# SeanNaren/deepspeech.pytorch

Measured on NVIDIA H100. Metric: utterances/sec (train step, 161x1000 spectrogram), higher is better.
Workload: dtype fp16-operands(rnn)+tf32(conv/fc)

## Files before the change

deepspeech.pytorch_b200/csrc/common.cuh:

```cuda
#pragma once
#include <cuda_runtime.h>
#include <stdint.h>
#include <stdio.h>
#include <string.h>
#include <atomic>

#include "../../include/ds2_b200.h"

namespace ds2 {

void set_error(const char* fmt, ...);
extern std::atomic<long long> g_launches;
int precision();
inline bool tensor_core_mode() { return precision() != DS2_PREC_FP32; }
inline bool f16_gemm_mode() { return precision() == DS2_PREC_F16; }

inline cudaStream_t as_stream(void* s) { return reinterpret_cast<cudaStream_t>(s); }

inline int current_device() {
  int d = 0;
  (void)cudaGetDevice(&d);
  return d & 63;
}
struct DeviceOnce {
  std::atomic<unsigned long long> mask{0};
  bool first() const { return !((mask.load(std::memory_order_acquire) >> current_device()) & 1ull); }
  void done() { mask.fetch_or(1ull << current_device(), std::memory_order_release); }
};
int device_sm_count();

void note_fallback(const char* what, int rnn, int T, int B, int H, int D);

extern std::atomic<void*> g_side_stream;
int side_wait_for_workspace(const void* ws, cudaStream_t main);
int side_fork(cudaStream_t main, cudaStream_t side);
int side_mark_workspace(const void* ws, cudaStream_t side);

#define DS2_CHECK_CUDA(expr)                                                             \
  do {                                                                                   \
    cudaError_t _e = (expr);                                                             \
    if (_e != cudaSuccess) {                                                             \
      ds2::set_error("%s:%d %s -> %s", __FILE__, __LINE__, #expr, cudaGetErrorString(_e)); \
      return DS2_ERR_CUDA;                                                               \
    }                                                                                    \
  } while (0)

#define DS2_REQUIRE(cond, ...)                      \
  do {                                              \
    if (!(cond)) {                                  \
      ds2::set_error(__VA_ARGS__);                  \
      return DS2_ERR_INVALID;                       \
    }                                               \
  } while (0)

#define DS2_LAUNCH(kernel, grid, block, smem, stream, ...)                \
  do {                                                                    \
    kernel<<<(grid), (block), (smem), (stream)>>>(__VA_ARGS__);           \
    ds2::g_launches.fetch_add(1, std::memory_order_relaxed);              \
    DS2_CHECK_CUDA(cudaGetLastError());                                   \
  } while (0)

void prof_begin(const char* tag, cudaStream_t st);
void prof_end(cudaStream_t st);
struct ProfRange {
  cudaStream_t st;
  ProfRange(const char* tag, cudaStream_t s) : st(s) { prof_begin(tag, s); }
  ~ProfRange() { prof_end(st); }
};
#define DS2_PROF(tag, st) ds2::ProfRange _prof_range_##__LINE__(tag, st)

inline int cdiv(long long a, long long b) { return (int)((a + b - 1) / b); }
#ifdef __CUDACC__
__device__ __forceinline__ int cdiv_dev(int a, int b) { return (a + b - 1) / b; }
#endif
inline size_t align_up(size_t x, size_t a) { return (x + a - 1) / a * a; }

template <typename T>
inline T* carve(void* base, size_t& off, size_t bytes) {
  T* at = base ? reinterpret_cast<T*>(static_cast<char*>(base) + off) : nullptr;
  off += align_up(bytes, 256);
  return at;
}

#ifdef __CUDACC__
__device__ __forceinline__ float sigmoidf_(float x) { return 1.0f / (1.0f + expf(-x)); }

__device__ __forceinline__ float warp_sum(float v) {
#pragma unroll
  for (int o = 16; o > 0; o >>= 1) v += __shfl_xor_sync(0xffffffffu, v, o);
  return v;
}
__device__ __forceinline__ double warp_sum_d(double v) {
#pragma unroll
  for (int o = 16; o > 0; o >>= 1) v += __shfl_xor_sync(0xffffffffu, v, o);
  return v;
}
#endif

int gemm_simt(int transA, int transB, int M, int N, int K, float alpha, const float* A, int lda, const float* B,
              int ldb, float beta, float* C, int ldc, cudaStream_t st, void* ws = nullptr, size_t ws_bytes = 0);
size_t gemm_simt_workspace_bytes(int M, int N, int K);
int gemm_tc(int transA, int transB, int M, int N, int K, float alpha, const float* A, int lda, const float* B,
            int ldb, float beta, float* C, int ldc, void* ws, size_t ws_bytes, cudaStream_t st);
size_t gemm_tc_workspace_bytes(int transA, int transB, int M, int N, int K);
int gemm_tc_f16(int M, int N, int K, float alpha, const void* A16, int lda, const void* B16, int ldb, float beta,
                float* C, int ldc, const float* alpha_dev, cudaStream_t st);
int f32_to_f16_rows(int rows, int cols, const float* in, size_t ld_in, void* out, size_t ld_out, const float* scale_dev,
                    cudaStream_t st);
int f32_to_f16_transpose(int rows, int cols, const float* in, size_t ld_in, void* out, size_t ld_out, void* outT,
                         size_t ld_outT, const float* scale_dev, cudaStream_t st);
int pow2_scale_for(int rows, int cols, const float* x, size_t ld, unsigned int* absmax_ws, float* scale, int top,
                   cudaStream_t st);

int bn_rows_fwd(int rows, int F, const float* x, const float* gamma, const float* beta, float* rmean, float* rvar,
                int training, float momentum, float eps, float* y, float* xhat, float* mean_invstd ,
                double* ws_sums , cudaStream_t st);
int bn_rows_reapply(int rows, int F, const float* x, const float* gamma, const float* beta,
                    const float* mean_invstd, float* y, float* xhat, cudaStream_t st);
int transpose(int R, int C, const float* in, float* out, cudaStream_t st);
int transpose_strided(int R, int C, const float* in, size_t ldi, float* out, size_t ldo, cudaStream_t st);
int bn_rows_bwd(int rows, int F, const float* xhat, const float* gamma, const float* mean_invstd, const float* dy,
                float* dx, float* dgamma, float* dbeta, double* ws_sums , cudaStream_t st);

}
```

deepspeech.pytorch_b200/csrc/conv_frontend.cu:

```cuda
#include <stdlib.h>

#include "common.cuh"

namespace ds2 {

constexpr int CO = 32;
constexpr int TD = 4, TT = 64;

template <int KH, int KW, int SH, int SW>
struct ConvGeom {
  static constexpr int ROWS = (TD - 1) * SH + KH;
  static constexpr int XIN = (4 - 1) * SW + KW;
  static constexpr int XVEC = (XIN + 3) / 4;
  static constexpr int COLS = ((15 * 4 * SW + XVEC * 4) + 3) / 4 * 4;
  static constexpr int SLAB = ROWS * COLS;
  static constexpr int WTS = KH * KW * CO;
  static constexpr size_t SMEM = (size_t)(SLAB + WTS) * sizeof(float);
};

template <int KH, int KW, int SH, int SW>
__global__ void __launch_bounds__(256) conv_fwd_kernel(const float* __restrict__ in, int Cin, int Hin, int Win,
                                                       const float* __restrict__ wpk, const float* __restrict__ bias,
                                                       float* __restrict__ out, int Hout, int Wout, size_t ob,
                                                       size_t oc, size_t orow, int PH, int PW,
// ... 230 lines not shown
    du_dz[base + i] = v;
  }
  __shared__ float red[8];
  float s = warp_sum(v);
  if (threadIdx.x % 32 == 0) red[threadIdx.x / 32] = s;
  __syncthreads();
  if (threadIdx.x == 0) {
    float tot = 0.f;
    for (int w = 0; w < (int)blockDim.x / 32; ++w) tot += red[w];
    dbias_part[((size_t)c * B + b) * gridDim.x + blockIdx.x] = tot;
  }
}

__global__ void ordered_sum_kernel(int n, const float* __restrict__ part, float* __restrict__ out) {
  __shared__ float red[256];
  const float* p = part + (size_t)blockIdx.x * n;
  float s = 0.f;
  for (int i = threadIdx.x; i < n; i += 256) s += p[i];
  red[threadIdx.x] = s;
  __syncthreads();
  for (int w = 128; w > 0; w >>= 1) {
    if (threadIdx.x < w) red[threadIdx.x] += red[threadIdx.x + w];
    __syncthreads();
  }
  if (threadIdx.x == 0) out[blockIdx.x] = red[0];
}

__global__ void bn_bwd_params2d_kernel(const double* __restrict__ sums, float* __restrict__ dgamma,
                                       float* __restrict__ dbeta) {
  int c = threadIdx.x;
  if (c < CO) { dbeta[c] = (float)sums[c]; dgamma[c] = (float)sums[CO + c]; }
}

__global__ void __launch_bounds__(256) conv2_dw_kernel(int B, int T, const float* __restrict__ dz2,
                                                       const float* __restrict__ a1, float* __restrict__ dw2) {
  constexpr int D1 = DS2_CONV1_D, D2 = DS2_CONV2_D, TW = 64, AW = TW + 12;
  __shared__ __align__(16) float dsm[TW][36];
  __shared__ float asmx[AW][33];
  const int kh = blockIdx.x, b = blockIdx.y, tid = threadIdx.x;
  const int cog = tid / 32, ci = tid % 32;
  float acc[4][11];
#pragma unroll
  for (int c = 0; c < 4; ++c)
#pragma unroll
    for (int k = 0; k < 11; ++k) acc[c][k] = 0.f;
  for (int d = 0; d < D2; ++d) {
    const int r = 2 * d + kh - 10;
    if (r < 0 || r >= D1) continue;
    for (int t0 = 0; t0 < T; t0 += TW) {
      for (int idx = tid; idx < CO * TW; idx += 256) {
        int tt = idx % TW, co = idx / TW, t = t0 + tt;
        dsm[tt][co] = (t < T) ? dz2[(((size_t)b * CO + co) * D2 + d) * T + t] : 0.f;
      }
      for (int idx = tid; idx < CO * AW; idx += 256) {
        int tt = idx % AW, c2 = idx / AW, t = t0 + tt - 5;
        asmx[tt][c2] = (t >= 0 && t < T) ? a1[(((size_t)b * CO + c2) * D1 + r) * T + t] : 0.f;
      }
      __syncthreads();
#pragma unroll 1
      for (int tb = 0; tb < TW; tb += 4) {
        float win[14];
#pragma unroll
        for (int i = 0; i < 14; ++i) win[i] = asmx[tb + i][ci];
#pragma unroll
        for (int j = 0; j < 4; ++j) {
          float4 dv = *reinterpret_cast<const float4*>(&dsm[tb + j][cog * 4]);
#pragma unroll
          for (int k = 0; k < 11; ++k) {
            float a = win[j + k];
            acc[0][k] = fmaf(dv.x, a, acc[0][k]); acc[1][k] = fmaf(dv.y, a, acc[1][k]);
            acc[2][k] = fmaf(dv.z, a, acc[2][k]); acc[3][k] = fmaf(dv.w, a, acc[3][k]);
          }
        }
      }
      __syncthreads();
    }
  }
#pragma unroll
  for (int c = 0; c < 4; ++c)
#pragma unroll
    for (int k = 0; k < 11; ++k)
      atomicAdd(&dw2[((((size_t)(cog * 4 + c)) * CO + ci) * 21 + kh) * 11 + k], acc[c][k]);
}

constexpr int C1_KG = 14, C1_TW = 64, C1_XW = 2 * C1_TW + 12, C1_DSPLIT = 6;
__global__ void __launch_bounds__(128) conv1_dw_kernel(int B, int Tin, int T, const float* __restrict__ dz1,
                                                       const float* __restrict__ x, float* __restrict__ dw1) {
  constexpr int D1 = DS2_CONV1_D, F = DS2_NUM_FREQ, TW = C1_TW, XW = C1_XW;
  __shared__ __align__(16) float dsm[TW][CO];
  __shared__ float xsm[C1_KG][XW];
  const int kh0 = blockIdx.x * C1_KG, b = blockIdx.y, tid = threadIdx.x;
  const int dper = (D1 + C1_DSPLIT - 1) / C1_DSPLIT, d0 = blockIdx.z * dper, d1 = min(D1, d0 + dper);
  const int cog = tid % 8, khl = tid / 8, kh = kh0 + khl;
  const bool worker = khl < C1_KG && kh < 41;
  const int khr = worker ? khl : 0;
  float acc[4][11];
#pragma unroll
  for (int c = 0; c < 4; ++c)
#pragma unroll
    for (int k = 0; k < 11; ++k) acc[c][k] = 0.f;
  for (int d = d0; d < d1; ++d) {
    for (int t0 = 0; t0 < T; t0 += TW) {
      for (int idx = tid; idx < CO * TW; idx += 128) {
        const int tt = idx % TW, c2 = idx / TW, t = t0 + tt;
        dsm[tt][c2] = (t < T) ? dz1[(((size_t)b * CO + c2) * D1 + d) * T + t] : 0.f;
      }
      for (int idx = tid; idx < C1_KG * XW; idx += 128) {
        const int cc = idx % XW, kl = idx / XW, r = 2 * d + kh0 + kl - 20, c = 2 * t0 + cc - 5;
        xsm[kl][cc] = (kh0 + kl < 41 && r >= 0 && r < F && c >= 0 && c < Tin) ? x[((size_t)b * F + r) * Tin + c] : 0.f;
      }
      __syncthreads();
      if (worker) {
#pragma unroll 1
        for (int tb = 0; tb < TW; tb += 4) {
          float win[17];
#pragma unroll
          for (int i = 0; i < 17; ++i) win[i] = xsm[khr][2 * tb + i];
#pragma unroll
          for (int j = 0; j < 4; ++j) {
            const float4 dv = *reinterpret_cast<const float4*>(&dsm[tb + j][cog * 4]);
#pragma unroll
            for (int k = 0; k < 11; ++k) {
              const float a = win[2 * j + k];
              acc[0][k] = fmaf(dv.x, a, acc[0][k]); acc[1][k] = fmaf(dv.y, a, acc[1][k]);
              acc[2][k] = fmaf(dv.z, a, acc[2][k]); acc[3][k] = fmaf(dv.w, a, acc[3][k]);
            }
          }
        }
      }
      __syncthreads();
    }
  }
  if (worker) {
#pragma unroll
    for (int c = 0; c < 4; ++c)
#pragma unroll
      for (int k = 0; k < 11; ++k) atomicAdd(&dw1[((size_t)(cog * 4 + c) * 41 + kh) * 11 + k], acc[c][k]);
  }
}

template <int KH, int KW, int SH, int SW>
static int launch_conv(const float* in, int B, int Cin, int Hin, int Win, const float* wpk, const float* bias,
                       float* out, int Hout, int Wout, size_t ob, size_t oc, size_t orow, int PH, int PW,
                       const int32_t* out_len, double* sums, cudaStream_t st) {
  using Gm = ConvGeom<KH, KW, SH, SW>;
  auto kern = conv_fwd_kernel<KH, KW, SH, SW>;
  DS2_CHECK_CUDA(cudaFuncSetAttribute(kern, cudaFuncAttributeMaxDynamicSharedMemorySize, (int)Gm::SMEM));
  dim3 grid(cdiv(Wout, TT), cdiv(Hout, TD), B);
  DS2_LAUNCH(kern, grid, 256, Gm::SMEM, st, in, Cin, Hin, Win, wpk, bias, out, Hout, Wout, ob, oc, orow, PH, PW,
             out_len, sums);
  return DS2_OK;
}

int conv_tc_run(const float* in_cl, int B, int T, int R_in, int R_out, const float* taps, int n_taps, int J,
                int row_mul, int row_off, int row_step, int w_off, int w_step, float* out, size_t ob, size_t oc,
                size_t orow, int out_row_mul, int out_row_off, const float* bias, const int32_t* out_len,
                double* stat_sums, cudaStream_t st);
int nchw_to_cl(int B, int R, int T, const float* in, float* out, cudaStream_t st);
int pack_conv2_tc(const float* w2, float* wn_fwd, float* wd_bwd, cudaStream_t st);
int conv2_wgrad_tc(const float* dz2, const float* a1, float* a1_shifted, float* part, int B, int T, float* dw2,
                   cudaStream_t st);
int conv1_wgrad_tc(const float* dz1, const float* x, float* xs, float* part, int B, int T, int Tp, float* dw1,
                   cudaStream_t st);
size_t conv_wgrad_tc_partial_floats();

struct ConvWs {
  float *wpk1, *wpk2, *wTe, *wTo, *du2, *da1;
  float *taps_f, *taps_b, *cl;
  float* shifted;
  float* wg_part;
  float* db_part;
  double* sums;
};
static size_t conv_ws_carve(int B, int T, void* base, ConvWs& w) {
  const size_t Tp = (size_t)(T - 1) / 2 + 1;
  size_t off = 0;
  w.wpk1 = carve<float>(base, off, (size_t)41 * 11 * CO * 4);
  w.wpk2 = carve<float>(base, off, (size_t)CO * 21 * 11 * CO * 4);
  w.wTe = carve<float>(base, off, (size_t)CO * 11 * 11 * CO * 4);
  w.wTo = carve<float>(base, off, (size_t)CO * 10 * 11 * CO * 4);
  w.sums = carve<double>(base, off, 4 * 64 * sizeof(double));
  w.du2 = carve<float>(base, off, (size_t)B * CO * DS2_CONV2_D * Tp * 4);
  w.da1 = carve<float>(base, off, (size_t)B * CO * DS2_CONV1_D * Tp * 4);
  w.taps_f = carve<float>(base, off, (size_t)21 * 352 * 32 * 4);
  w.taps_b = carve<float>(base, off, (size_t)21 * 352 * 32 * 4);
  w.cl = carve<float>(base, off, (size_t)B * CO * DS2_CONV1_D * Tp * 4);
  w.shifted = carve<float>(base, off, (size_t)4 * B * CO * DS2_CONV1_D * (Tp + 4) * 4);
  w.wg_part = carve<float>(base, off, conv_wgrad_tc_partial_floats() * 4);
  w.db_part = carve<float>(base, off, (size_t)CO * B * cdiv((long long)DS2_CONV1_D * Tp, 256) * 4);
  return off;
}

}

extern "C" {
using namespace ds2;

size_t ds2_conv_frontend_workspace_bytes(int B, int T) {
  if (B <= 0 || T <= 0) return 0;
  ConvWs w;
  return conv_ws_carve(B, T, nullptr, w) + 256;
}

int ds2_conv_frontend_fwd(int B, int T, const float* x, const int32_t* out_len, const float* w1, const float* b1,
                          const float* g1, const float* be1, float* rm1, float* rv1, const float* w2,
                          const float* b2, const float* g2, const float* be2, float* rm2, float* rv2, int training,
                          float momentum, float eps, float* y, float* z1, float* a1, float* z2, float* stats,
                          void* ws, size_t ws_bytes, void* stream) {
  DS2_REQUIRE(B > 0 && T > 0, "conv fwd: bad shape B=%d T=%d", B, T);
  DS2_REQUIRE(ws_bytes >= ds2_conv_frontend_workspace_bytes(B, T), "conv fwd: workspace too small");
  cudaStream_t st = as_stream(stream);
  const int Tp = (T - 1) / 2 + 1, D1 = DS2_CONV1_D, D2 = DS2_CONV2_D, F = DS2_NUM_FREQ;
  ConvWs W;
  conv_ws_carve(B, T, ws, W);
  DS2_PROF("conv_fwd", st);
  DS2_CHECK_CUDA(cudaMemsetAsync(W.sums, 0, 4 * 64 * sizeof(double), st));
  DS2_LAUNCH(pack_fwd_kernel, cdiv(41 * 11 * CO, 256), 256, 0, st, 1, 41, 11, w1, W.wpk1);
  DS2_LAUNCH(pack_fwd_kernel, cdiv(CO * 21 * 11 * CO, 256), 256, 0, st, CO, 21, 11, w2, W.wpk2);
  int rc = launch_conv<41, 11, 2, 2>(x, B, 1, F, T, W.wpk1, b1, z1, D1, Tp, (size_t)CO * D1 * Tp, (size_t)D1 * Tp,
                                     (size_t)Tp, 20, 5, out_len, training ? W.sums : nullptr, st);
  if (rc) return rc;
  DS2_LAUNCH(bn2d_finalize_kernel, 1, 32, 0, st, (double)B * D1 * Tp, W.sums, g1, be1, rm1, rv1, training, momentum,
             eps, stats);
  DS2_LAUNCH(bn_act_kernel, 132 * 8, 256, 0, st, B, D1, Tp, z1, stats, g1, be1, out_len, a1);
  if (tensor_core_mode()) {
    rc = nchw_to_cl(B, D1, Tp, a1, W.cl, st);
    if (rc) return rc;
    rc = pack_conv2_tc(w2, W.taps_f, nullptr, st);
    if (rc) return rc;
    rc = conv_tc_run(W.cl, B, Tp, D1, D2, W.taps_f, 21, 21, 2, -10, 1, 0, 1, z2, (size_t)CO * D2 * Tp, (size_t)D2 * Tp,
                     (size_t)Tp, 1, 0, b2, out_len, training ? W.sums + 64 : nullptr, st);
  } else {
    rc = launch_conv<21, 11, 2, 1>(a1, B, CO, D1, Tp, W.wpk2, b2, z2, D2, Tp, (size_t)CO * D2 * Tp, (size_t)D2 * Tp,
                                   (size_t)Tp, 10, 5, out_len, training ? W.sums + 64 : nullptr, st);
  }
  if (rc) return rc;
  DS2_LAUNCH(bn2d_finalize_kernel, 1, 32, 0, st, (double)B * D2 * Tp, W.sums + 64, g2, be2, rm2, rv2, training,
             momentum, eps, stats + 64);
  DS2_LAUNCH(bn_act_transpose_kernel, dim3(cdiv(Tp, 32), cdiv(CO * D2, 32), B), dim3(32, 8), 0, st, B, D2, Tp, z2,
             stats + 64, g2, be2, out_len, y);
  return DS2_OK;
}

int ds2_conv_frontend_bwd(int B, int T, const float* x, const int32_t* out_len, const float* w1, const float* g1,
                          const float* be1, const float* w2, const float* g2, const float* be2, const float* z1,
                          const float* a1, const float* z2, const float* stats, const float* dy, float* dw1,
                          float* db1, float* dg1, float* dbe1, float* dw2, float* db2, float* dg2, float* dbe2,
                          void* ws, size_t ws_bytes, void* stream) {
  DS2_REQUIRE(B > 0 && T > 0, "conv bwd: bad shape B=%d T=%d", B, T);
  DS2_REQUIRE(ws_bytes >= ds2_conv_frontend_workspace_bytes(B, T), "conv bwd: workspace too small");
  (void)w1;
  cudaStream_t st = as_stream(stream);
  const int Tp = (T - 1) / 2 + 1, D1 = DS2_CONV1_D, D2 = DS2_CONV2_D;
  ConvWs W;
  conv_ws_carve(B, T, ws, W);
  double* s2 = W.sums + 128;
  double* s1 = W.sums + 192;
  DS2_PROF("conv_bwd", st);
  DS2_CHECK_CUDA(cudaMemsetAsync(s2, 0, 128 * sizeof(double), st));
  DS2_CHECK_CUDA(cudaMemsetAsync(db2, 0, CO * sizeof(float), st));
  DS2_CHECK_CUDA(cudaMemsetAsync(db1, 0, CO * sizeof(float), st));
  DS2_CHECK_CUDA(cudaMemsetAsync(dw2, 0, sizeof(float) * CO * CO * 21 * 11, st));
  DS2_CHECK_CUDA(cudaMemsetAsync(dw1, 0, sizeof(float) * CO * 41 * 11, st));

  DS2_LAUNCH(bn_bwd_reduce_kernel<true>, dim3(cdiv(Tp, 32), cdiv(CO * D2, 32), B), dim3(32, 8), 0, st, B, D2, Tp, z2,
             stats + 64, g2, be2, out_len, dy, W.du2, s2);
  DS2_LAUNCH(bn_bwd_params2d_kernel, 1, 32, 0, st, s2, dg2, dbe2);
  DS2_LAUNCH(bn_bwd_apply_kernel, dim3(cdiv(D2 * Tp, 256), CO, B), 256, 0, st, B, D2, Tp, 1.0 / ((double)B * D2 * Tp),
             z2, stats + 64, g2, out_len, s2, W.du2, W.db_part);
  DS2_LAUNCH(ordered_sum_kernel, CO, 256, 0, st, B * cdiv(D2 * Tp, 256), W.db_part, db2);
  cudaStream_t side = as_stream(g_side_stream.load());
  bool forked = false;
  {
    int wrc = 1;
    if (tensor_core_mode()) {
      cudaStream_t wst = st;
      if (side && Tp % 4 == 0) {
        int frc = side_fork(st, side);
        if (frc) return frc;
        wst = side;
        forked = true;
      }
      wrc = conv2_wgrad_tc(W.du2, a1, W.shifted, W.wg_part, B, Tp, dw2, wst);
      if (wrc < 0) return wrc;
      if (forked) {
        int mrc = side_mark_workspace(ws, side);
        if (mrc) return mrc;
      }
    }
    if (wrc == 1) DS2_LAUNCH(conv2_dw_kernel, dim3(21, B), 256, 0, st, B, Tp, W.du2, a1, dw2);
  }
  DS2_LAUNCH(pack_bwd_data_kernel, cdiv(CO * 11 * 11 * CO, 256), 256, 0, st, 0, w2, W.wTe);
  DS2_LAUNCH(pack_bwd_data_kernel, cdiv(CO * 10 * 11 * CO, 256), 256, 0, st, 1, w2, W.wTo);
  const size_t ob = (size_t)CO * D1 * Tp, oc = (size_t)D1 * Tp;
  int rc;
  if (tensor_core_mode()) {
    rc = nchw_to_cl(B, D2, Tp, W.du2, W.cl, st);
    if (rc) return rc;
    rc = pack_conv2_tc(w2, nullptr, W.taps_b, st);
    if (rc) return rc;
    rc = conv_tc_run(W.cl, B, Tp, D2, 41, W.taps_b, 21, 11, 1, 5, -1, 0, 2, W.da1, ob, oc, (size_t)Tp, 2, 0, nullptr,
                     nullptr, nullptr, st);
    if (rc) return rc;
    rc = conv_tc_run(W.cl, B, Tp, D2, 40, W.taps_b, 21, 10, 1, 5, -1, 1, 2, W.da1, ob, oc, (size_t)Tp, 2, 1, nullptr,
                     nullptr, nullptr, st);
    if (rc) return rc;
  } else {
    rc = launch_conv<11, 11, 1, 1>(W.du2, B, CO, D2, Tp, W.wTe, nullptr, W.da1, 41, Tp, ob, oc, (size_t)2 * Tp, 5, 5,
                                   nullptr, nullptr, st);
    if (rc) return rc;
    rc = launch_conv<10, 11, 1, 1>(W.du2, B, CO, D2, Tp, W.wTo, nullptr, W.da1 + Tp, 40, Tp, ob, oc, (size_t)2 * Tp, 4, 5,
                                   nullptr, nullptr, st);
    if (rc) return rc;
  }
  DS2_LAUNCH(bn_bwd_reduce_kernel<false>, dim3(cdiv(Tp, 32), cdiv(CO * D1, 32), B), dim3(32, 8), 0, st, B, D1, Tp,
             z1, stats, g1, be1, out_len, W.da1, W.da1, s1);
  DS2_LAUNCH(bn_bwd_params2d_kernel, 1, 32, 0, st, s1, dg1, dbe1);
  DS2_LAUNCH(bn_bwd_apply_kernel, dim3(cdiv(D1 * Tp, 256), CO, B), 256, 0, st, B, D1, Tp, 1.0 / ((double)B * D1 * Tp),
             z1, stats, g1, out_len, s1, W.da1, W.db_part);
  DS2_LAUNCH(ordered_sum_kernel, CO, 256, 0, st, B * cdiv(D1 * Tp, 256), W.db_part, db1);
  if (forked) {
    int jrc = side_wait_for_workspace(ws, st);
    if (jrc) return jrc;
  }
  {
    int wrc = 1;
    if (tensor_core_mode()) {
      wrc = conv1_wgrad_tc(W.da1, x, W.shifted, W.wg_part, B, T, Tp, dw1, st);
      if (wrc < 0) return wrc;
    }
    if (wrc == 1) DS2_LAUNCH(conv1_dw_kernel, dim3(3, B, C1_DSPLIT), 128, 0, st, B, T, Tp, W.da1, x, dw1);
  }
  return DS2_OK;
}

}
```

deepspeech.pytorch_b200/csrc/conv_tc.cu:

```cuda
#include "common.cuh"
#include "tc_common.cuh"

namespace ds2 {
int make_tmap_4d_f32(CUtensorMap* out, const float* base, const unsigned long long dims[4],
                     const unsigned long long strides_bytes[3], const unsigned int box[4]);
int make_tmap_nd_f32(CUtensorMap* out, const float* base, int rank, const unsigned long long* dims,
                     const unsigned long long* strides_bytes, const unsigned int* box);

namespace cv {
constexpr int CH = 32, KW = 11, NN = KW * CH;
constexpr int MP = 64, TO = MP - (KW - 1);
constexpr int A_BYTES = MP * 128;
constexpr int W_HALF = (NN / 2) * 128;
constexpr int STAGE_BYTES = A_BYTES + 2 * W_HALF;
constexpr int STAGES = 3;
constexpr int OUT_LD = 33;
constexpr int THREADS = 384;
constexpr int SMEM_BYTES = 1024 + STAGES * STAGE_BYTES + (TO + 10) * OUT_LD * 4 + 256;
}

__device__ __forceinline__ void tma_load_4d_w(void* dst, const CUtensorMap* m, uint64_t* bar, int c0, int c1, int c2,
                                              int c3) {
  asm volatile(
      "{\n\t.reg .pred pe;\n\telect.sync _|pe, 0xffffffff;\n\t"
      "@pe cp.async.bulk.tensor.4d.shared::cluster.global.tile.mbarrier::complete_tx::bytes [%0], [%1, {%3, %4, %5, %6}], [%2];\n\t}"
      ::"r"(tc::smem_u32(dst)), "l"(reinterpret_cast<uint64_t>(m)), "r"(tc::smem_u32(bar)), "r"(c0), "r"(c1), "r"(c2),
        "r"(c3)
      : "memory");
}
__device__ __forceinline__ void tma_load_5d_w(void* dst, const CUtensorMap* m, uint64_t* bar, int c0, int c1, int c2,
                                              int c3, int c4) {
  asm volatile(
      "{\n\t.reg .pred pe;\n\telect.sync _|pe, 0xffffffff;\n\t"
      "@pe cp.async.bulk.tensor.5d.shared::cluster.global.tile.mbarrier::complete_tx::bytes [%0], [%1, {%3, %4, %5, %6, %7}], [%2];\n\t}"
      ::"r"(tc::smem_u32(dst)), "l"(reinterpret_cast<uint64_t>(m)), "r"(tc::smem_u32(bar)), "r"(c0), "r"(c1), "r"(c2),
        "r"(c3), "r"(c4)
      : "memory");
}

struct ConvTcParams {
  CUtensorMap tmA;
  CUtensorMap tmW;
  int B, T, R_in, R_out;
  int J;
  int row_mul, row_off, row_step;
  int w_off, w_step;
  float* out;
  size_t ob, oc, orow;
  int out_row_mul, out_row_off;
  const float* bias;
  const int32_t* out_len;
  double* stat_sums;
};

__global__ void __launch_bounds__(cv::THREADS, 1) conv_tc_kernel(const __grid_constant__ ConvTcParams p) {
  using namespace cv;
  using namespace tc;
  extern __shared__ uint8_t smem_raw[];
  uint8_t* smem = reinterpret_cast<uint8_t*>((reinterpret_cast<uintptr_t>(smem_raw) + 1023) & ~(uintptr_t)1023);
  float* out_s = reinterpret_cast<float*>(smem + STAGES * STAGE_BYTES);
  uint64_t* full = reinterpret_cast<uint64_t*>(out_s + (TO + 10) * OUT_LD);
  uint64_t* empty = full + STAGES;

  const int warp = threadIdx.x / 32, lane = threadIdx.x % 32;
  const int t0 = blockIdx.x * TO, d = blockIdx.y, b = blockIdx.z;

  int j_lo = 0, j_hi = p.J;
  {
    const int r0 = p.row_mul * d + p.row_off;
    while (j_lo < j_hi && (r0 + j_lo * p.row_step < 0 || r0 + j_lo * p.row_step >= p.R_in)) ++j_lo;
    while (j_hi > j_lo && (r0 + (j_hi - 1) * p.row_step < 0 || r0 + (j_hi - 1) * p.row_step >= p.R_in)) --j_hi;
  }
  const int nj = j_hi - j_lo;

  if (warp == 0 && lane == 0) {
    tma_prefetch_desc(&p.tmA);
    tma_prefetch_desc(&p.tmW);
    for (int i = 0; i < STAGES; ++i) { mbar_init(&full[i], 1); mbar_init(&empty[i], 2); }
    fence_barrier_init();
  }
  for (int i = threadIdx.x; i < (TO + 10) * OUT_LD; i += THREADS) out_s[i] = 0.f;
  __syncthreads();

  if (warp == 0) {
    int s = 0;
    uint32_t ph = 0;
    for (int jj = 0; jj < nj; ++jj) {
      const int j = j_lo + jj;
      const int r = p.row_mul * d + p.row_off + j * p.row_step;
      const int wi = p.w_off + j * p.w_step;
      mbar_wait(&empty[s], ph ^ 1);
      mbar_arrive_expect_tx_w(&full[s], (uint32_t)STAGE_BYTES);
      uint8_t* st = smem + s * STAGE_BYTES;
      tma_load_4d_w(st, &p.tmA, &full[s], 0, t0 - 5, r, b);
      tma_load_3d_w(st + A_BYTES, &p.tmW, &full[s], 0, 0, wi);
      tma_load_3d_w(st + A_BYTES + W_HALF, &p.tmW, &full[s], 0, NN / 2, wi);
      if (++s == STAGES) { s = 0; ph ^= 1; }
    }
  } else if (warp >= 4 && nj > 0) {
    const int wg = warp / 4 - 1;
    float acc[NN / 4];
#pragma unroll
    for (int i = 0; i < NN / 4; ++i) acc[i] = 0.f;
    int s = 0;
    uint32_t ph = 0;
    for (int jj = 0; jj < nj; ++jj) {
      mbar_wait(&full[s], ph);
      const uint64_t ad = smem_desc_sw128(smem_u32(smem + s * STAGE_BYTES));
      const uint64_t bd = smem_desc_sw128(smem_u32(smem + s * STAGE_BYTES + A_BYTES + wg * W_HALF));
      wg_fence();
#pragma unroll
      for (int k = 0; k < 4; ++k) Wgmma<NN / 2, false>::mma(acc, ad + (uint64_t)(2 * k), bd + (uint64_t)(2 * k), 1u);
      wg_release(&empty[s]);
      if (++s == STAGES) { s = 0; ph ^= 1; }
    }
    const int w = warp % 4;
#pragma unroll
    for (int kw = 0; kw < KW; ++kw) {
#pragma unroll
      for (int i = 0; i < NN / 16; ++i) {
        const bool in0 = (i >> 2) == kw, in1 = ((NN / 16 + i) >> 2) == kw;
        if (!in0 && !in1) continue;
        if (wg == 0 ? !in0 : !in1) continue;
#pragma unroll
        for (int e = 0; e < 4; ++e) {
          const int pl = 16 * w + (lane >> 2) + 8 * (e >> 1);
          const int n = NN / 2 * wg + 8 * i + 2 * (lane & 3) + (e & 1);
          const int to = pl - kw;
          if (to >= 0 && to < TO) out_s[to * OUT_LD + n % CH] += acc[4 * i + e];
        }
      }
      asm volatile("bar.sync 1, 256;" ::: "memory");
    }
  }
  __syncthreads();
  if (warp >= 4 && warp < 8) {
    const int q = warp % 4;
    const int L = p.out_len ? p.out_len[b] : p.T;
    const int orow_idx = p.out_row_mul * d + p.out_row_off;
    for (int cc = 0; cc < 8; ++cc) {
      const int c = q * 8 + cc;
      const float bv = p.bias ? p.bias[c] : 0.f;
      float* op = p.out + (size_t)b * p.ob + (size_t)c * p.oc + (size_t)orow_idx * p.orow;
      float s1 = 0.f, s2 = 0.f;
      for (int to = lane; to < TO; to += 32) {
        const int t = t0 + to;
        if (t < p.T) {
          const float val = (t < L) ? out_s[to * OUT_LD + c] + bv : 0.f;
          op[t] = val;
          s1 += val;
          s2 = fmaf(val, val, s2);
        }
      }
      if (p.stat_sums) {
        s1 = warp_sum(s1);
        s2 = warp_sum(s2);
        if (lane == 0) {
          atomicAdd(&p.stat_sums[c], (double)s1);
          atomicAdd(&p.stat_sums[CH + c], (double)s2);
        }
      }
    }
  }
}

__global__ void pack_conv2_tc_fwd_kernel(const float* __restrict__ w2, float* __restrict__ wn) {
  int i = blockIdx.x * blockDim.x + threadIdx.x, n = 21 * cv::NN * 32;
  if (i >= n) return;
  int ci = i % 32, nn = (i / 32) % cv::NN, kh = i / (32 * cv::NN);
  int kw = nn / 32, co = nn % 32;
  wn[i] = w2[(((size_t)co * 32 + ci) * 21 + kh) * 11 + kw];
}
__global__ void pack_conv2_tc_bwd_kernel(const float* __restrict__ w2, float* __restrict__ wd) {
  int i = blockIdx.x * blockDim.x + threadIdx.x, n = 21 * cv::NN * 32;
  if (i >= n) return;
  int co = i % 32, nn = (i / 32) % cv::NN, kh = i / (32 * cv::NN);
  int kwi = nn / 32, ci = nn % 32;
  wd[i] = w2[(((size_t)co * 32 + ci) * 21 + kh) * 11 + (10 - kwi)];
}

__global__ void nchw_to_cl_kernel(int R, int T, const float* __restrict__ in, float* __restrict__ out) {
  __shared__ float tile[32][33];
  const int b = blockIdx.z, r = blockIdx.y, t0 = blockIdx.x * 32;
  for (int c = threadIdx.y; c < 32; c += 8) {
    int t = t0 + threadIdx.x;
    tile[c][threadIdx.x] = (t < T) ? in[(((size_t)b * 32 + c) * R + r) * T + t] : 0.f;
  }
  __syncthreads();
  for (int j = threadIdx.y; j < 32; j += 8) {
    int t = t0 + j;
    if (t < T) out[(((size_t)b * R + r) * T + t) * 32 + threadIdx.x] = tile[threadIdx.x][j];
  }
}

int nchw_to_cl(int B, int R, int T, const float* in, float* out, cudaStream_t st) {
  DS2_LAUNCH(nchw_to_cl_kernel, dim3(cdiv(T, 32), R, B), dim3(32, 8), 0, st, R, T, in, out);
  return DS2_OK;
}

int pack_conv2_tc(const float* w2, float* wn_fwd, float* wd_bwd, cudaStream_t st) {
  const int n = 21 * cv::NN * 32;
  if (wn_fwd) DS2_LAUNCH(pack_conv2_tc_fwd_kernel, cdiv(n, 256), 256, 0, st, w2, wn_fwd);
  if (wd_bwd) DS2_LAUNCH(pack_conv2_tc_bwd_kernel, cdiv(n, 256), 256, 0, st, w2, wd_bwd);
  return DS2_OK;
}

static int make_tmap_cl(CUtensorMap* out, const float* base, int T, int R, int B);

int conv_tc_run(const float* in_cl, int B, int T, int R_in, int R_out, const float* taps, int n_taps, int J,
                int row_mul, int row_off, int row_step, int w_off, int w_step, float* out, size_t ob, size_t oc,
                size_t orow, int out_row_mul, int out_row_off, const float* bias, const int32_t* out_len,
                double* stat_sums, cudaStream_t st) {
  ConvTcParams p{};
  int rc = make_tmap_cl(&p.tmA, in_cl, T, R_in, B);
  if (rc) return rc;
  rc = make_tmap_3d(&p.tmW, taps, 32, cv::NN, n_taps, 32, (size_t)32 * cv::NN, 32, cv::NN / 2, 1);
  if (rc) return rc;
  p.B = B; p.T = T; p.R_in = R_in; p.R_out = R_out; p.J = J;
  p.row_mul = row_mul; p.row_off = row_off; p.row_step = row_step; p.w_off = w_off; p.w_step = w_step;
  p.out = out; p.ob = ob; p.oc = oc; p.orow = orow; p.out_row_mul = out_row_mul; p.out_row_off = out_row_off;
  p.bias = bias; p.out_len = out_len; p.stat_sums = stat_sums;
  static DeviceOnce attr_once;
  if (attr_once.first()) {
    DS2_CHECK_CUDA(cudaFuncSetAttribute(conv_tc_kernel, cudaFuncAttributeMaxDynamicSharedMemorySize, cv::SMEM_BYTES));
    attr_once.done();
  }
  dim3 grid(cdiv(T, cv::TO), R_out, B);
  DS2_LAUNCH(conv_tc_kernel, grid, cv::THREADS, cv::SMEM_BYTES, st, p);
  return DS2_OK;
}

namespace wg {
constexpr int KT = 32;
constexpr int KH = 21;
constexpr int KH_PER = 2;
constexpr int GROUPS = 6;
constexpr int A_BYTES = KH_PER * 32 * 128;
constexpr int B_BYTES = cv::NN * 128;
constexpr int STAGE_BYTES = A_BYTES + B_BYTES;
constexpr int STAGES = 3;
constexpr int THREADS = 384;
constexpr int SMEM_BYTES = 1024 + STAGES * STAGE_BYTES + 256;
}

struct WgradParams {
  CUtensorMap tmDz;
  CUtensorMap tmS4;
  CUtensorMap tmS2;
  CUtensorMap tmS1;
  int B, T, slices;
  float* part;
};
__constant__ int KW_OF_BLOCK[11] = {1, 0, 5, 4, 3, 2, 9, 8, 7, 6, 10};

__global__ void shift_copies_kernel(size_t rows, int T, const float* __restrict__ a1, float* __restrict__ a1r) {
  const int Tp = T + 4;
  size_t i = (size_t)blockIdx.x * blockDim.x + threadIdx.x, n = rows * Tp, stride = (size_t)gridDim.x * blockDim.x;
  for (; i < n; i += stride) {
    const int t = (int)(i % Tp);
    const float* src = a1 + (i / Tp) * T;
#pragma unroll
    for (int sft = 0; sft <= 3; ++sft) {
      const int ts = t - sft;
      a1r[(size_t)sft * n + i] = (ts >= 0 && ts < T) ? src[ts] : 0.f;
    }
  }
}

__global__ void __launch_bounds__(wg::THREADS, 1) conv2_wgrad_tc_kernel(const __grid_constant__ WgradParams p) {
  using namespace wg;
  using namespace tc;
  extern __shared__ uint8_t smem_raw[];
  uint8_t* smem = reinterpret_cast<uint8_t*>((reinterpret_cast<uintptr_t>(smem_raw) + 1023) & ~(uintptr_t)1023);
  uint64_t* full = reinterpret_cast<uint64_t*>(smem + STAGES * STAGE_BYTES);
  uint64_t* empty = full + STAGES;
  const int warp = threadIdx.x / 32, lane = threadIdx.x % 32;
  const int parity = blockIdx.x / GROUPS, kh0 = parity + 2 * KH_PER * (blockIdx.x % GROUPS);
  if (kh0 >= KH) return;
  const int nkh = min(KH_PER, (KH - 1 - kh0) / 2 + 1);
  const int nr = (DS2_CONV1_D - parity + 1) / 2;
  const int pairs = p.B * nr;
  const int per = (pairs + (int)gridDim.y - 1) / (int)gridDim.y;
  const int p0 = blockIdx.y * per, p1 = min(pairs, p0 + per);
  const int nkt = (p.T + KT - 1) / KT;
  auto row_active = [&](int r) {
    const int d_hi = (r + 10 - kh0) / 2, d_lo = (r + 10 - (kh0 + 2 * (nkh - 1))) / 2;
    return d_hi >= 0 && d_lo < DS2_CONV2_D;
  };

  if (warp == 0 && lane == 0) {
    tma_prefetch_desc(&p.tmDz);
    tma_prefetch_desc(&p.tmS4);
    for (int i = 0; i < STAGES; ++i) { mbar_init(&full[i], 1); mbar_init(&empty[i], 2); }
    fence_barrier_init();
  }
  __syncthreads();

  int nchunks = 0;
  for (int pi = p0; pi < p1; ++pi)
    if (row_active(2 * (pi % nr) + parity)) nchunks += nkt;

  if (warp == 0) {
    int s = 0;
    uint32_t ph = 0;
    for (int pi = p0; pi < p1; ++pi) {
      const int b = pi / nr, r = 2 * (pi % nr) + parity;
      if (!row_active(r)) continue;
      for (int kt = 0; kt < nkt; ++kt) {
        mbar_wait(&empty[s], ph ^ 1);
        mbar_arrive_expect_tx_w(&full[s], (uint32_t)(nkh * 32 * 128 + cv::NN * 128));
        uint8_t* st = smem + s * STAGE_BYTES;
        for (int i = 0; i < nkh; ++i)
          tma_load_4d_w(st + i * 4096, &p.tmDz, &full[s], kt * KT, (r + 10 - kh0) / 2 - i, 0, b);
        uint8_t* nb = st + A_BYTES;
        tma_load_5d_w(nb, &p.tmS2, &full[s], kt * KT - 4, r, 0, b, 0);
        tma_load_5d_w(nb + 2 * 4096, &p.tmS4, &full[s], kt * KT, r, 0, b, 0);
        tma_load_5d_w(nb + 6 * 4096, &p.tmS4, &full[s], kt * KT + 4, r, 0, b, 0);
        tma_load_5d_w(nb + 10 * 4096, &p.tmS1, &full[s], kt * KT + 8, r, 0, b, 3);
        if (++s == STAGES) { s = 0; ph ^= 1; }
      }
    }
  } else if (warp >= 4) {
    const int wg = warp / 4 - 1;
    float acc[cv::NN / 4];
#pragma unroll
    for (int i = 0; i < cv::NN / 4; ++i) acc[i] = 0.f;
    int s = 0;
    uint32_t ph = 0;
    for (int c = 0; c < nchunks; ++c) {
      mbar_wait(&full[s], ph);
      const uint64_t ad = smem_desc_sw128(smem_u32(smem + s * STAGE_BYTES));
      const uint64_t bd = smem_desc_sw128(smem_u32(smem + s * STAGE_BYTES + A_BYTES + wg * cv::W_HALF));
      wg_fence();
#pragma unroll
      for (int k = 0; k < 4; ++k) Wgmma<cv::NN / 2, false>::mma(acc, ad + (uint64_t)(2 * k), bd + (uint64_t)(2 * k), 1u);
      wg_release(&empty[s]);
      if (++s == STAGES) { s = 0; ph ^= 1; }
    }
    const int w = warp % 4;
    float* tile = p.part + ((size_t)blockIdx.x * gridDim.y + blockIdx.y) * 64 * cv::NN;
#pragma unroll
    for (int i = 0; i < cv::NN / 16; ++i) {
#pragma unroll
      for (int hh = 0; hh < 2; ++hh) {
        const int m = 16 * w + (lane >> 2) + 8 * hh;
        const int n = cv::NN / 2 * wg + 8 * i + 2 * (lane & 3);
        *reinterpret_cast<float2*>(tile + (size_t)m * cv::NN + n) = make_float2(acc[4 * i + 2 * hh], acc[4 * i + 2 * hh + 1]);
      }
    }
  }
}

__global__ void conv2_wgrad_reduce_kernel(int slices, const float* __restrict__ part, float* __restrict__ dw2) {
  using namespace wg;
  const int idx = blockIdx.x * blockDim.x + threadIdx.x;
  if (idx >= 32 * 32 * KH * cv::KW) return;
  const int kw = idx % cv::KW, kh = (idx / cv::KW) % KH, ci = (idx / (cv::KW * KH)) % 32, co = idx / (cv::KW * KH * 32);
  const int parity = kh & 1, q = (kh - parity) / 2, x = parity * GROUPS + q / KH_PER, m = 32 * (q % KH_PER) + co;
  int blk = 0;
  while (KW_OF_BLOCK[blk] != kw) ++blk;
  const float* src = part + (size_t)x * slices * 64 * cv::NN + (size_t)m * cv::NN + blk * 32 + ci;
  float s = 0.f;
  for (int y = 0; y < slices; ++y) s += src[(size_t)y * 64 * cv::NN];
  dw2[idx] = s;
}

int conv2_wgrad_tc(const float* dz2, const float* a1, float* a1_shifted , float* part,
                   int B, int T, float* dw2, cudaStream_t st) {
  if (T % 4 != 0) return 1;
  WgradParams p{};
  {
    const size_t rows = (size_t)B * 32 * 81;
    DS2_LAUNCH(shift_copies_kernel, device_sm_count() * 8, 256, 0, st, rows, T, a1, a1_shifted);
    const unsigned long long Tq = (unsigned long long)T + 4;
    unsigned long long dims[5] = {Tq, 81ull, 32ull, (unsigned long long)B, 4ull};
    unsigned long long str[4] = {Tq * 4, 81ull * Tq * 4, 32ull * 81 * Tq * 4, (unsigned long long)rows * Tq * 4};
    unsigned int box[5] = {32u, 1u, 32u, 1u, 4u};
    int rc = make_tmap_nd_f32(&p.tmS4, a1_shifted, 5, dims, str, box);
    if (rc) return rc;
    box[4] = 2u;
// ... 208 lines not shown
```

Measured before the change: 632.1.

## Make conv tensor-core kernel persistent with ping-pong consumer warpgroups

```diff
diff --git a/deepspeech.pytorch_b200/csrc/common.cuh b/deepspeech.pytorch_b200/csrc/common.cuh
--- a/deepspeech.pytorch_b200/csrc/common.cuh
+++ b/deepspeech.pytorch_b200/csrc/common.cuh
@@ -28,6 +28,10 @@
   void done() { mask.fetch_or(1ull << current_device(), std::memory_order_release); }
 };
 int device_sm_count();
+
+struct ConvRows {
+  int R_out, J, row_off, w_off, out_row_off;
+};
 
 void note_fallback(const char* what, int rnn, int T, int B, int H, int D);
 
diff --git a/deepspeech.pytorch_b200/csrc/conv_frontend.cu b/deepspeech.pytorch_b200/csrc/conv_frontend.cu
--- a/deepspeech.pytorch_b200/csrc/conv_frontend.cu
+++ b/deepspeech.pytorch_b200/csrc/conv_frontend.cu
@@ -406,10 +406,9 @@
   return DS2_OK;
 }
 
-int conv_tc_run(const float* in_cl, int B, int T, int R_in, int R_out, const float* taps, int n_taps, int J,
-                int row_mul, int row_off, int row_step, int w_off, int w_step, float* out, size_t ob, size_t oc,
-                size_t orow, int out_row_mul, int out_row_off, const float* bias, const int32_t* out_len,
-                double* stat_sums, cudaStream_t st);
+int conv_tc_run(const float* in_cl, int B, int T, int R_in, const float* taps, int n_taps, int row_mul, int row_step,
+                int w_step, int out_row_mul, const ConvRows* rows, int n_classes, float* out, size_t ob, size_t oc,
+                size_t orow, const float* bias, const int32_t* out_len, double* stat_sums, cudaStream_t st);
 int nchw_to_cl(int B, int R, int T, const float* in, float* out, cudaStream_t st);
 int pack_conv2_tc(const float* w2, float* wn_fwd, float* wd_bwd, cudaStream_t st);
 int conv2_wgrad_tc(const float* dz2, const float* a1, float* a1_shifted, float* part, int B, int T, float* dw2,
@@ -482,8 +481,9 @@
     if (rc) return rc;
     rc = pack_conv2_tc(w2, W.taps_f, nullptr, st);
     if (rc) return rc;
-    rc = conv_tc_run(W.cl, B, Tp, D1, D2, W.taps_f, 21, 21, 2, -10, 1, 0, 1, z2, (size_t)CO * D2 * Tp, (size_t)D2 * Tp,
-                     (size_t)Tp, 1, 0, b2, out_len, training ? W.sums + 64 : nullptr, st);
+    const ConvRows rows = {D2, 21, -10, 0, 0};
+    rc = conv_tc_run(W.cl, B, Tp, D1, W.taps_f, 21, 2, 1, 1, 1, &rows, 1, z2, (size_t)CO * D2 * Tp, (size_t)D2 * Tp,
+                     (size_t)Tp, b2, out_len, training ? W.sums + 64 : nullptr, st);
   } else {
     rc = launch_conv<21, 11, 2, 1>(a1, B, CO, D1, Tp, W.wpk2, b2, z2, D2, Tp, (size_t)CO * D2 * Tp, (size_t)D2 * Tp,
                                    (size_t)Tp, 10, 5, out_len, training ? W.sums + 64 : nullptr, st);
@@ -553,11 +553,9 @@
     if (rc) return rc;
     rc = pack_conv2_tc(w2, nullptr, W.taps_b, st);
     if (rc) return rc;
-    rc = conv_tc_run(W.cl, B, Tp, D2, 41, W.taps_b, 21, 11, 1, 5, -1, 0, 2, W.da1, ob, oc, (size_t)Tp, 2, 0, nullptr,
-                     nullptr, nullptr, st);
-    if (rc) return rc;
-    rc = conv_tc_run(W.cl, B, Tp, D2, 40, W.taps_b, 21, 10, 1, 5, -1, 1, 2, W.da1, ob, oc, (size_t)Tp, 2, 1, nullptr,
-                     nullptr, nullptr, st);
+    const ConvRows rows[2] = {{41, 11, 5, 0, 0}, {40, 10, 5, 1, 1}};
+    rc = conv_tc_run(W.cl, B, Tp, D2, W.taps_b, 21, 1, -1, 2, 2, rows, 2, W.da1, ob, oc, (size_t)Tp, nullptr, nullptr,
+                     nullptr, st);
     if (rc) return rc;
   } else {
     rc = launch_conv<11, 11, 1, 1>(W.du2, B, CO, D2, Tp, W.wTe, nullptr, W.da1, 41, Tp, ob, oc, (size_t)2 * Tp, 5, 5,
diff --git a/deepspeech.pytorch_b200/csrc/conv_tc.cu b/deepspeech.pytorch_b200/csrc/conv_tc.cu
--- a/deepspeech.pytorch_b200/csrc/conv_tc.cu
+++ b/deepspeech.pytorch_b200/csrc/conv_tc.cu
@@ -14,9 +14,11 @@
 constexpr int W_HALF = (NN / 2) * 128;
 constexpr int STAGE_BYTES = A_BYTES + 2 * W_HALF;
 constexpr int STAGES = 3;
-constexpr int OUT_LD = 33;
+constexpr int OUT_LD = 33, OUT_FLOATS = TO * OUT_LD;
 constexpr int THREADS = 384;
-constexpr int SMEM_BYTES = 1024 + STAGES * STAGE_BYTES + (TO + 10) * OUT_LD * 4 + 256;
+constexpr int PRODUCER_REGS = 40, MMA_REGS = 232;
+constexpr int ORDER_BAR = 1, EPI_BAR = 3;
+constexpr int SMEM_BYTES = 1024 + STAGES * STAGE_BYTES + 2 * OUT_FLOATS * 4 + 256;
 }
 
 __device__ __forceinline__ void tma_load_4d_w(void* dst, const CUtensorMap* m, uint64_t* bar, int c0, int c1, int c2,
@@ -41,113 +43,157 @@
 struct ConvTcParams {
   CUtensorMap tmA;
   CUtensorMap tmW;
-  int B, T, R_in, R_out;
-  int J;
-  int row_mul, row_off, row_step;
-  int w_off, w_step;
+  int B, T, R_in;
+  int ntt;
+  ConvRows rows[2];
+  int tiles0, tiles;
+  int row_mul, row_step, w_step, out_row_mul;
   float* out;
   size_t ob, oc, orow;
-  int out_row_mul, out_row_off;
   const float* bias;
   const int32_t* out_len;
   double* stat_sums;
 };
+
+struct ConvTile {
+  int t0, d, b, cls, j_lo, nj;
+};
+__device__ __forceinline__ ConvTile conv_tile(const ConvTcParams& p, int u) {
+  ConvTile t;
+  t.cls = u >= p.tiles0;
+  if (t.cls) u -= p.tiles0;
+  const ConvRows& rc = p.rows[t.cls];
+  t.t0 = (u % p.ntt) * cv::TO;
+  u /= p.ntt;
+  t.d = u % rc.R_out;
+  t.b = u / rc.R_out;
+  int j_lo = 0, j_hi = rc.J;
+  const int r0 = p.row_mul * t.d + rc.row_off;
+  while (j_lo < j_hi && (r0 + j_lo * p.row_step < 0 || r0 + j_lo * p.row_step >= p.R_in)) ++j_lo;
+  while (j_hi > j_lo && (r0 + (j_hi - 1) * p.row_step < 0 || r0 + (j_hi - 1) * p.row_step >= p.R_in)) --j_hi;
+  t.j_lo = j_lo;
+  t.nj = j_hi - j_lo;
+  return t;
+}
+
+__device__ __forceinline__ void named_bar_sync(int id, int threads) {
+  asm volatile("bar.sync %0, %1;" ::"r"(id), "r"(threads) : "memory");
+}
+__device__ __forceinline__ void named_bar_arrive(int id, int threads) {
+  asm volatile("bar.arrive %0, %1;" ::"r"(id), "r"(threads) : "memory");
+}
 
 __global__ void __launch_bounds__(cv::THREADS, 1) conv_tc_kernel(const __grid_constant__ ConvTcParams p) {
   using namespace cv;
   using namespace tc;
   extern __shared__ uint8_t smem_raw[];
   uint8_t* smem = reinterpret_cast<uint8_t*>((reinterpret_cast<uintptr_t>(smem_raw) + 1023) & ~(uintptr_t)1023);
-  float* out_s = reinterpret_cast<float*>(smem + STAGES * STAGE_BYTES);
-  uint64_t* full = reinterpret_cast<uint64_t*>(out_s + (TO + 10) * OUT_LD);
+  float* out_s0 = reinterpret_cast<float*>(smem + STAGES * STAGE_BYTES);
+  uint64_t* full = reinterpret_cast<uint64_t*>(out_s0 + 2 * OUT_FLOATS);
   uint64_t* empty = full + STAGES;
 
   const int warp = threadIdx.x / 32, lane = threadIdx.x % 32;
-  const int t0 = blockIdx.x * TO, d = blockIdx.y, b = blockIdx.z;
-
-  int j_lo = 0, j_hi = p.J;
-  {
-    const int r0 = p.row_mul * d + p.row_off;
-    while (j_lo < j_hi && (r0 + j_lo * p.row_step < 0 || r0 + j_lo * p.row_step >= p.R_in)) ++j_lo;
-    while (j_hi > j_lo && (r0 + (j_hi - 1) * p.row_step < 0 || r0 + (j_hi - 1) * p.row_step >= p.R_in)) --j_hi;
-  }
-  const int nj = j_hi - j_lo;
 
   if (warp == 0 && lane == 0) {
     tma_prefetch_desc(&p.tmA);
     tma_prefetch_desc(&p.tmW);
-    for (int i = 0; i < STAGES; ++i) { mbar_init(&full[i], 1); mbar_init(&empty[i], 2); }
+    for (int i = 0; i < STAGES; ++i) { mbar_init(&full[i], 1); mbar_init(&empty[i], 1); }
     fence_barrier_init();
   }
-  for (int i = threadIdx.x; i < (TO + 10) * OUT_LD; i += THREADS) out_s[i] = 0.f;
   __syncthreads();
 
-  if (warp == 0) {
-    int s = 0;
-    uint32_t ph = 0;
-    for (int jj = 0; jj < nj; ++jj) {
-      const int j = j_lo + jj;
-      const int r = p.row_mul * d + p.row_off + j * p.row_step;
-      const int wi = p.w_off + j * p.w_step;
-      mbar_wait(&empty[s], ph ^ 1);
-      mbar_arrive_expect_tx_w(&full[s], (uint32_t)STAGE_BYTES);
-      uint8_t* st = smem + s * STAGE_BYTES;
-      tma_load_4d_w(st, &p.tmA, &full[s], 0, t0 - 5, r, b);
-      tma_load_3d_w(st + A_BYTES, &p.tmW, &full[s], 0, 0, wi);
-      tma_load_3d_w(st + A_BYTES + W_HALF, &p.tmW, &full[s], 0, NN / 2, wi);
-      if (++s == STAGES) { s = 0; ph ^= 1; }
-    }
-  } else if (warp >= 4 && nj > 0) {
-    const int wg = warp / 4 - 1;
-    float acc[NN / 4];
-#pragma unroll
-    for (int i = 0; i < NN / 4; ++i) acc[i] = 0.f;
-    int s = 0;
-    uint32_t ph = 0;
-    for (int jj = 0; jj < nj; ++jj) {
-      mbar_wait(&full[s], ph);
+  if (warp < 4) {
+    setmaxnreg_dec<PRODUCER_REGS>();
+    if (warp == 0) {
+      int g = 0;
+      for (int u = blockIdx.x; u < p.tiles; u += gridDim.x) {
+        const ConvTile t = conv_tile(p, u);
+        const ConvRows& rc = p.rows[t.cls];
+        for (int jj = 0; jj < t.nj; ++jj, ++g) {
+          const int j = t.j_lo + jj;
+          const int r = p.row_mul * t.d + rc.row_off + j * p.row_step;
+          const int wi = rc.w_off + j * p.w_step;
+          const int s = g % STAGES;
+          mbar_wait(&empty[s], ((g / STAGES) & 1) ^ 1);
+          mbar_arrive_expect_tx_w(&full[s], (uint32_t)STAGE_BYTES);
+          uint8_t* st = smem + s * STAGE_BYTES;
+          tma_load_4d_w(st, &p.tmA, &full[s], 0, t.t0 - 5, r, t.b);
+          tma_load_3d_w(st + A_BYTES, &p.tmW, &full[s], 0, 0, wi);
+          tma_load_3d_w(st + A_BYTES + W_HALF, &p.tmW, &full[s], 0, NN / 2, wi);
+        }
+      }
+    }
+    return;
+  }
+
+  setmaxnreg_inc<MMA_REGS>();
+  const int wg = warp / 4 - 1, w = warp % 4;
+  const bool leader = (threadIdx.x & 127) == 0;
+  float* out_s = out_s0 + wg * OUT_FLOATS;
+  int g = 0;
+  int i = 0;
+  for (int u = blockIdx.x; u < p.tiles; u += gridDim.x, ++i) {
+    const ConvTile t = conv_tile(p, u);
+    if ((i & 1) != wg) {
+      g += t.nj;
+      continue;
+    }
+    if (i > 0) named_bar_sync(ORDER_BAR + wg, 256);
+    float acc[NN / 2];
+#pragma unroll
+    for (int k = 0; k < NN / 2; ++k) acc[k] = 0.f;
+    for (int jj = 0; jj < t.nj; ++jj, ++g) {
+      const int s = g % STAGES;
+      mbar_wait(&full[s], (g / STAGES) & 1);
       const uint64_t ad = smem_desc_sw128(smem_u32(smem + s * STAGE_BYTES));
-      const uint64_t bd = smem_desc_sw128(smem_u32(smem + s * STAGE_BYTES + A_BYTES + wg * W_HALF));
+      const uint64_t bd = smem_desc_sw128(smem_u32(smem + s * STAGE_BYTES + A_BYTES));
       wg_fence();
 #pragma unroll
-      for (int k = 0; k < 4; ++k) Wgmma<NN / 2, false>::mma(acc, ad + (uint64_t)(2 * k), bd + (uint64_t)(2 * k), 1u);
-      wg_release(&empty[s]);
-      if (++s == STAGES) { s = 0; ph ^= 1; }
-    }
-    const int w = warp % 4;
+      for (int k = 0; k < 4; ++k) {
+#pragma unroll
+        for (int h = 0; h < 2; ++h)
+          Wgmma<NN / 2, false>::mma(acc + (NN / 4) * h, ad + (uint64_t)(2 * k),
+                                    bd + (uint64_t)(W_HALF / 16 * h + 2 * k), 1u);
+      }
+      wg_commit();
+      wg_wait<1>();
+      if (jj > 0 && leader) mbar_arrive(&empty[(g - 1) % STAGES]);
+    }
+    if (u + (int)gridDim.x < p.tiles) named_bar_arrive(ORDER_BAR + (wg ^ 1), 256);
+    wg_wait<0>();
+    if (t.nj > 0 && leader) mbar_arrive(&empty[(g - 1) % STAGES]);
+
+    named_bar_sync(EPI_BAR + wg, 128);
 #pragma unroll
     for (int kw = 0; kw < KW; ++kw) {
 #pragma unroll
-      for (int i = 0; i < NN / 16; ++i) {
-        const bool in0 = (i >> 2) == kw, in1 = ((NN / 16 + i) >> 2) == kw;
-        if (!in0 && !in1) continue;
-        if (wg == 0 ? !in0 : !in1) continue;
+      for (int ib = 4 * kw; ib < 4 * kw + 4; ++ib) {
 #pragma unroll
         for (int e = 0; e < 4; ++e) {
           const int pl = 16 * w + (lane >> 2) + 8 * (e >> 1);
-          const int n = NN / 2 * wg + 8 * i + 2 * (lane & 3) + (e & 1);
+          const int co = 8 * (ib % 4) + 2 * (lane & 3) + (e & 1);
           const int to = pl - kw;
-          if (to >= 0 && to < TO) out_s[to * OUT_LD + n % CH] += acc[4 * i + e];
+          if (to >= 0 && to < TO) {
+            float* o = out_s + to * OUT_LD + co;
+            *o = (kw == 0 ? 0.f : *o) + acc[4 * ib + e];
+          }
         }
       }
-      asm volatile("bar.sync 1, 256;" ::: "memory");
-    }
-  }
-  __syncthreads();
-  if (warp >= 4 && warp < 8) {
-    const int q = warp % 4;
-    const int L = p.out_len ? p.out_len[b] : p.T;
-    const int orow_idx = p.out_row_mul * d + p.out_row_off;
+      named_bar_sync(EPI_BAR + wg, 128);
+    }
+
+    const int L = p.out_len ? p.out_len[t.b] : p.T;
+    const int orow_idx = p.out_row_mul * t.d + p.rows[t.cls].out_row_off;
     for (int cc = 0; cc < 8; ++cc) {
-      const int c = q * 8 + cc;
+      const int c = w * 8 + cc;
       const float bv = p.bias ? p.bias[c] : 0.f;
-      float* op = p.out + (size_t)b * p.ob + (size_t)c * p.oc + (size_t)orow_idx * p.orow;
+      float* op = p.out + (size_t)t.b * p.ob + (size_t)c * p.oc + (size_t)orow_idx * p.orow;
       float s1 = 0.f, s2 = 0.f;
       for (int to = lane; to < TO; to += 32) {
-        const int t = t0 + to;
-        if (t < p.T) {
-          const float val = (t < L) ? out_s[to * OUT_LD + c] + bv : 0.f;
-          op[t] = val;
+        const int tt = t.t0 + to;
+        if (tt < p.T) {
+          const float val = (tt < L) ? out_s[to * OUT_LD + c] + bv : 0.f;
+          op[tt] = val;
           s1 += val;
           s2 = fmaf(val, val, s2);
         }
@@ -207,25 +253,30 @@
 
 static int make_tmap_cl(CUtensorMap* out, const float* base, int T, int R, int B);
 
-int conv_tc_run(const float* in_cl, int B, int T, int R_in, int R_out, const float* taps, int n_taps, int J,
-                int row_mul, int row_off, int row_step, int w_off, int w_step, float* out, size_t ob, size_t oc,
-                size_t orow, int out_row_mul, int out_row_off, const float* bias, const int32_t* out_len,
-                double* stat_sums, cudaStream_t st) {
+int conv_tc_run(const float* in_cl, int B, int T, int R_in, const float* taps, int n_taps, int row_mul, int row_step,
+                int w_step, int out_row_mul, const ConvRows* rows, int n_classes, float* out, size_t ob, size_t oc,
+                size_t orow, const float* bias, const int32_t* out_len, double* stat_sums, cudaStream_t st) {
   ConvTcParams p{};
   int rc = make_tmap_cl(&p.tmA, in_cl, T, R_in, B);
   if (rc) return rc;
   rc = make_tmap_3d(&p.tmW, taps, 32, cv::NN, n_taps, 32, (size_t)32 * cv::NN, 32, cv::NN / 2, 1);
   if (rc) return rc;
-  p.B = B; p.T = T; p.R_in = R_in; p.R_out = R_out; p.J = J;
-  p.row_mul = row_mul; p.row_off = row_off; p.row_step = row_step; p.w_off = w_off; p.w_step = w_step;
-  p.out = out; p.ob = ob; p.oc = oc; p.orow = orow; p.out_row_mul = out_row_mul; p.out_row_off = out_row_off;
+  p.B = B; p.T = T; p.R_in = R_in; p.ntt = cdiv(T, cv::TO);
+  p.tiles = 0;
+  for (int c = 0; c < n_classes; ++c) {
+    p.rows[c] = rows[c];
+    p.tiles += p.ntt * rows[c].R_out * B;
+    if (c == 0) p.tiles0 = p.tiles;
+  }
+  p.row_mul = row_mul; p.row_step = row_step; p.w_step = w_step; p.out_row_mul = out_row_mul;
+  p.out = out; p.ob = ob; p.oc = oc; p.orow = orow;
   p.bias = bias; p.out_len = out_len; p.stat_sums = stat_sums;
   static DeviceOnce attr_once;
   if (attr_once.first()) {
     DS2_CHECK_CUDA(cudaFuncSetAttribute(conv_tc_kernel, cudaFuncAttributeMaxDynamicSharedMemorySize, cv::SMEM_BYTES));
     attr_once.done();
   }
-  dim3 grid(cdiv(T, cv::TO), R_out, B);
+  const int grid = p.tiles < device_sm_count() ? p.tiles : device_sm_count();
   DS2_LAUNCH(conv_tc_kernel, grid, cv::THREADS, cv::SMEM_BYTES, st, p);
   return DS2_OK;
 }
```

New measurement: 657.3, median of 6. 4.0% higher.
